# aokomoriuta/ConjugateGradient

Hardware: AMD Instinct MI355X
Metric: CG iterations/sec (7-pt Poisson 512^3); SpMV achieved HBM GB/s in roofline (higher is better)
Workload: dtype f64

## Files before the change

### conjugategradient_amd/csrc/common.hpp

```cpp
#pragma once
#include <hip/hip_runtime.h>
#include <cstddef>
#include <cstdint>
#include <cstdio>
#include <cstdarg>
#include <cstring>
#include <cmath>
#include <atomic>
#include <mutex>
#include <string>
#include <type_traits>
#include <vector>

#pragma GCC visibility push(default)
#include "../../include/MgcgGpu.h"
#pragma GCC visibility pop

namespace mgcg {

constexpr int kWave = 64;
constexpr int kBlock = 256;
constexpr int kNumXcd = 8;
constexpr int kNumCu = 256;
constexpr int kMaxGrid = kNumCu * 8;
// ... 580 lines not shown
void lsqr_enqueue_v(const LsqrRun& R, const FinalizeArgs& f, int k, int nUU);
int lsqr_enqueue_close_residual(const LsqrRun& R);
int lsqr_enqueue_close_normal(const LsqrRun& R);

int launch_cheb_start(hipStream_t s, const double* r, const double* dinv, double* d, double* z, long long n, double it,
                      double* partials, double* partialsZ, bool withRz);
void launch_cheb_init_scalars(hipStream_t s, const double* partials, int n, const double* partialsZ, int nZ, bool reduceFirst, const FinalizeArgs& f);
int launch_cheb_first(hipStream_t s, const FinalizeArgs& f, double* r, const double* Ap, const double* dinv, double* d, double* z, long long n, double it,
                      double* partials, double* partialsZ, bool withRz, const double* pApPartials, int nPAp);
void launch_cheb_finalize(hipStream_t s, const double* partials, int n, const double* partialsZ, int nZ, bool reduceFirst, const FinalizeArgs& f);
void launch_gershgorin(hipStream_t s, const double* elements, const int* rowOffsets, long long nnz, long long n, const double* dinv, double* partials, double* out);

void launch_jacobi_setup(hipStream_t s, const double* elements, const int* rowOffsets, const int* columnIndeces, long long nnz, long long n, long long rowBase,
                         double* dinv, int* bad );

struct FinalizeArgs {
    CgScalars* sc;
    HostMirror* mirror;
    double* trace; int traceCap;
    double tol; int minIt; int maxIt; int rule;
    int preconditioned;
};
struct StopDecision { double res, shown; bool stop; int status; };
__device__ __forceinline__ StopDecision decide_stop(const FinalizeArgs& f, double rrNew, double inf, double rr0, int it)
{
    StopDecision d;
    d.res = sqrt(rrNew);
    if (f.rule == MGCG_RULE_HANDMADECL) d.res = inf;
    d.shown = d.res;
    bool converged;
    switch (f.rule) {
    case MGCG_RULE_NATIVE:   converged = (f.minIt <= it) && (d.res < f.tol); break;
    case MGCG_RULE_SIMPLE:   converged = (f.minIt < it) && (d.res < f.tol); break;
    case MGCG_RULE_VIENNACL: d.shown = sqrt(rrNew / rr0); converged = (f.minIt < it) && (rrNew / rr0 < f.tol * f.tol); break;
    default:                 converged = (it >= f.minIt) && (it <= f.maxIt) && (d.res < f.tol); break;
    }
    d.status = MGCG_OK;
    d.stop = converged;
    if (!d.stop && it >= f.minIt && it > f.maxIt) { d.stop = true; d.status = MGCG_MAXIT_EXCEEDED; }
    if (!d.stop && !(d.res == d.res && fabs(d.res) <= 1.79e308)) { d.stop = true; d.status = MGCG_NONFINITE; }
    return d;
}
void launch_reduce_to(hipStream_t s, const double* partials, int n, double* dst, const int* done);
void launch_reduce2_to(hipStream_t s, const double* pA, int nA, double* dstA, const double* pB, int nB, double* dstB, const int* done);
void launch_finalize(hipStream_t s, const double* partials, const double* partialsInf, int n, bool reduceFirst, const FinalizeArgs& f);
void launch_finalize_precond(hipStream_t s, const double* partials, int n, bool reduceFirst, CgScalars* sc);
void launch_init_scalars(hipStream_t s, const double* partials, const double* partialsZ, int n, bool reduceFirst, CgScalars* sc, HostMirror* mirror);

void launch_jacobi_first(hipStream_t s, long long n, double omega, const double* dinv, int dinvUniform, double dinvScalar, const double* b, double* x, const int* done);
void launch_uniform_check(hipStream_t s, const double* v, long long n, int* flag);
void launch_restrict(hipStream_t s, int nx, int ny, int nz, const double* r, double* bc, const int* done);
void launch_prolong_add(hipStream_t s, int nx, int ny, int nz, double* x, const double* e, const int* done);
void launch_prolong_linear_add(hipStream_t s, int nx, int ny, int nz, int z0, int z1, double* x, const double* eFull, const int* done);
void launch_restrict_linear(hipStream_t s, int nx, int ny, int nz, int z0, int z1, const double* rFull, double* bc, const int* done);
void launch_prolong_scaled(hipStream_t s, int nx, int ny, int nz, double* x, const double* b, double inner, double outer, const double* e, const int* done);
void launch_extract_dinv(hipStream_t s, const double* elements, const int* rowOffsets, const int* columnIndeces,
                         long long n, long long rowBase, double* dinv);
void launch_galerkin(hipStream_t s, int nx, int ny, int nz, int zBegin, int zEnd, const double* elements, const int* rowOffsets, const int* columnIndeces,
                     double sigma, const int* rowOffsetsC, int* countsC, double* elementsC, int* columnIndecesC, int* errFlag);
void launch_poisson(hipStream_t s, int nx, int ny, int nz, int zBegin, int zEnd, double* elements, int* rowOffsets, int* columnIndeces);
void launch_rebase(hipStream_t s, int* rowOffsets, long long n, int base);
long long poisson_nnz_host(int nx, int ny, int nz, int zBegin, int zEnd);
void launch_minmax_int(hipStream_t s, const int* v, long long n, int* out2 );
void launch_halo_rows(hipStream_t s, const int* rowOffsets, const int* columnIndeces, long long n, long long offset, int* out2 );

void launch_amg_restrict(hipStream_t s, long long nc, const int* aggOffsets, const int* members, const double* r, double* bc, const int* done);
void launch_amg_prolong_add(hipStream_t s, long long n, const int* agg, double* x, const double* e, const int* done);
void launch_amg_check_diagonal(hipStream_t s, const double* elements, const int* rowOffsets, const int* columnIndeces, long long n, int* badRow);
void launch_amg_row_max(hipStream_t s, const double* elements, const int* rowOffsets, const int* columnIndeces, long long n, double* rowMax);
void launch_amg_match_round(hipStream_t s, const double* elements, const int* rowOffsets, const int* columnIndeces, long long n, double theta,
                            const double* rowMax, int* match, int* pick, int* flags2);
void launch_amg_galerkin_count(hipStream_t s, long long nc, const int* aggOffsets, const int* members, const int* rowOffsets, const int* columnIndeces,
                               const int* agg, const int* expandOffsets, int* scratch, int* counts);
void launch_amg_galerkin_fill(hipStream_t s, long long nc, const int* aggOffsets, const int* members, const double* elements, const int* rowOffsets,
                              const int* columnIndeces, const int* agg, const int* expandOffsets, const int* scratch, const int* rowOffsetsC, double sigma,
                              double* elementsC, int* columnIndecesC);
void launch_amg_gather_values(hipStream_t s, long long m, const int* source, const double* elements, double* out);

constexpr int kTransposeShortMax = 32;
constexpr int kTransposeLdsMax = 4096;
void launch_transpose_check_offsets(hipStream_t s, const int* rowOffsets, long long rows, int* status3);
void launch_transpose_count(hipStream_t s, const int* rowOffsets, const int* columnIndeces, long long rows, long long columns, long long nnz, int* counts, int* badRow);
bool launch_transpose_claim_and_sort(hipStream_t s, const int* rowOffsets, const int* columnIndeces, long long rows, long long columns, long long nnz,
                                     const int* offsetsT, int* cursor, int* work, unsigned long long* keys);
void launch_transpose_emit(hipStream_t s, long long nnz, const unsigned long long* keys, const double* elements, int* outColumns, int* outSource, double* outElements);
void launch_transpose_merged(hipStream_t s, const int* rowOffsets, const int* columnIndeces, const int* offsetsT, const unsigned long long* keys, long long n, long long nnz,
                             int* mergedOffsets, int* mergedColumns, int* mergedSource);
void preload_kernels_transpose();

void launch_gs_colour_round(hipStream_t s, const int* rowOffsets, const int* columnIndeces, long long n, const int* colourIn, int* colourOut, int* flags, int* badRow);
void launch_gs_check(hipStream_t s, const int* rowOffsets, const int* columnIndeces, long long n, const int* colour, int* badRow);
void launch_gs_zero(hipStream_t s, long long n, double* x, const int* done);
void launch_gs_sweep(hipStream_t s, const int* rows, int count, const double* elements, const int* rowOffsets, const int* columnIndeces,
                     const double* b, const double* dinv, double omega, double* x, double avgRow, const int* done);
void preload_kernels_gs();

void launch_ilu_check_rows(hipStream_t s, const int* rowOffsets, const int* columnIndeces, long long n, int* flags3);
void launch_ilu_lengths(hipStream_t s, const int* rowOffsets, const int* rowOf, long long n, int* lengths);
void launch_ilu_build(hipStream_t s, const double* elements, const int* rowOffsets, const int* columnIndeces, const int* rowOf, const int* newOf, long long n,
                      double shift, const int* offsetsB, double* valuesB, int* columnsB, int* diagPos, int* dupRow, int lanes);
void launch_ilu_factor(hipStream_t s, int row0, int count, const int* offsetsB, const int* columnsB, const int* diagPos, double* valuesB, double* pinv,
                       const int* rowOf, int* badRow, int lanes);
int launch_ilu_pivot_range(hipStream_t s, const double* valuesB, const int* diagPos, long long n, double* partials);
void launch_ilu_pass(hipStream_t s, bool backward, int row0, int count, const double* valuesB, const int* offsetsB, const int* columnsB, const int* diagPos,
                     const double* pinv, const int* rowOf, const double* r, double* y, double* t, double* z, int lanes, const int* done);
void preload_kernels_ilu();
// ... 23 lines not shown
```

### conjugategradient_amd/csrc/kernels_mg.hip

```cpp
#include "common.hpp"

namespace mgcg {

static inline int grid1(long long n)
{
    long long b = (n + kBlock - 1) / kBlock;
    if (b > kMaxGrid) b = kMaxGrid;
    if (b < 1) b = 1;
    return (int)b;
}

typedef double d2mg __attribute__((ext_vector_type(2)));

template <bool UNIFORM>
__global__ __launch_bounds__(kBlock) void jacobi_first_kernel(long long n, double omega, const double* __restrict__ dinv, double dscalar,
                                                              const double* __restrict__ b, double* __restrict__ x, const int* done)
{
    if (done != nullptr && *done != 0) return;
    const bool wide = ((((uintptr_t)b) | ((uintptr_t)x) | ((uintptr_t)dinv)) & 15) == 0;
    if (wide) {
        const long long n2 = n >> 1;
        const long long per = ((n2 + gridDim.x - 1) / gridDim.x + (kBlock - 1)) & ~(long long)(kBlock - 1);
        long long end = per * (blockIdx.x + 1);
        end = end < n2 ? end : n2;
// ... 99 lines not shown
    const long long pairsL = (long long)(nx / 2) * ny * nz;
    if (pairsL <= 0 || pairsL >= 0x7fffffffLL) return false;
    const unsigned half = (unsigned)nx / 2, pairs = (unsigned)pairsL;
    auto lg = [](unsigned v) { int l = 0; while ((1u << l) < v) ++l; return ((1u << l) == v) ? l : -1; };
    const int lgHalf = lg(half), lgNy = lg((unsigned)ny);
    const bool pow2 = lgHalf >= 0 && lgNy >= 0;
    const int cy = ny > 1 ? 2 : 1, cz = nz > 1 ? 2 : 1;
    const unsigned NX = half, NY = (unsigned)(ny / cy);
    const int grid = grid1((long long)pairs);
#define GO(S, P) hipLaunchKernelGGL((prolong_pairs_kernel<S, P>), dim3(grid), dim3(kBlock), 0, s, half, (unsigned)ny, lgHalf, lgNy, cy, cz, NX, NY, pairs, x, b, inner, outer, e, done)
    if (scaled) { if (pow2) GO(true, true); else GO(true, false); }
    else { if (pow2) GO(false, true); else GO(false, false); }
#undef GO
    return true;
}

void launch_prolong_add(hipStream_t s, int nx, int ny, int nz, double* x, const double* e, const int* done)
{
    if (launch_prolong_pairs(s, false, nx, ny, nz, x, x, 0.0, 0.0, e, done)) return;
    hipLaunchKernelGGL(prolong_add_kernel, dim3(grid1((long long)nx * ny * nz)), dim3(kBlock), 0, s, nx, ny, nz, x, e, done);
}

__global__ __launch_bounds__(kBlock) void prolong_scaled_kernel(int nx, int ny, int nz, double* __restrict__ x, const double* __restrict__ b,
                                                                double inner, double outer, const double* __restrict__ e, const int* done)
{
    if (done != nullptr && *done != 0) return;
    const int cx = nx > 1 ? 2 : 1, cy = ny > 1 ? 2 : 1, cz = nz > 1 ? 2 : 1;
    const int NX = nx / cx, NY = ny / cy;
    const long long N = (long long)nx * ny * nz;
    const long long stride = (long long)gridDim.x * kBlock;
    for (long long i = (long long)blockIdx.x * kBlock + threadIdx.x; i < N; i += stride) {
        const int xx = (int)(i % nx), yy = (int)((i / nx) % ny), zz = (int)(i / ((long long)nx * ny));
        const double t = inner * b[i];
        const double x1 = outer * t;
        x[i] = x1 + e[((long long)(zz / cz) * NY + (yy / cy)) * NX + (xx / cx)];
    }
}
void launch_prolong_scaled(hipStream_t s, int nx, int ny, int nz, double* x, const double* b, double inner, double outer, const double* e, const int* done)
{
    if (launch_prolong_pairs(s, true, nx, ny, nz, x, b, inner, outer, e, done)) return;
    hipLaunchKernelGGL(prolong_scaled_kernel, dim3(grid1((long long)nx * ny * nz)), dim3(kBlock), 0, s, nx, ny, nz, x, b, inner, outer, e, done);
}

__device__ __forceinline__ int lin_terms(int i, int n, int idx[2], double w[2])
{
    if (n == 1) { idx[0] = 0; w[0] = 1.0; return 1; }
    const int I = i >> 1, J = (i & 1) ? I + 1 : I - 1;
    idx[0] = I; w[0] = 0.75;
    if (J < 0 || J >= (n >> 1)) return 1;
    idx[1] = J; w[1] = 0.25;
    return 2;
}

__global__ __launch_bounds__(kBlock) void prolong_linear_add_kernel(int nx, int ny, int nz, int z0, int z1, double* __restrict__ x,
                                                                    const double* __restrict__ eFull, const int* done)
{
    if (done != nullptr && *done != 0) return;
    const int NX = nx > 1 ? nx / 2 : 1, NY = ny > 1 ? ny / 2 : 1;
    const long long N = (long long)nx * ny * (z1 - z0);
    const long long stride = (long long)gridDim.x * kBlock;
    for (long long i = (long long)blockIdx.x * kBlock + threadIdx.x; i < N; i += stride) {
        const int xx = (int)(i % nx), yy = (int)((i / nx) % ny), zz = z0 + (int)(i / ((long long)nx * ny));
        int iz[2], iy[2], ix[2]; double wz[2], wy[2], wx[2];
        const int kz = lin_terms(zz, nz, iz, wz), ky = lin_terms(yy, ny, iy, wy), kx = lin_terms(xx, nx, ix, wx);
        double sum = 0.0;
        for (int a = 0; a < kz; ++a)
            for (int b = 0; b < ky; ++b) {
                const double wzy = wz[a] * wy[b];
                const long long base = ((long long)iz[a] * NY + iy[b]) * NX;
                for (int c = 0; c < kx; ++c) { const double w = wzy * wx[c]; const double t = w * eFull[base + ix[c]]; sum += t; }
            }
        x[i] = x[i] + sum;
    }
}
__global__ __launch_bounds__(kBlock) void prolong_linear_add_rows_kernel(int nx, int ny, int nz, int z0, int z1, int tx, double* __restrict__ x,
                                                                         const double* __restrict__ eFull, const int* done)
{
    if (done != nullptr && *done != 0) return;
    const int NX = nx >> 1, NY = ny > 1 ? ny / 2 : 1;
    const int ty = kBlock / tx;
    const int lx = threadIdx.x % tx, ly = threadIdx.x / tx;
    const long long rows = (long long)ny * (z1 - z0);
    const long long band = (rows + 7) / 8;
    const long long bandBegin = (blockIdx.x & 7) * band, bandEnd = bandBegin + band < rows ? bandBegin + band : rows;
    for (long long row = bandBegin + (long long)(blockIdx.x >> 3) * ty + ly; row < bandEnd; row += (long long)(gridDim.x >> 3) * ty) {
        const unsigned r32 = (unsigned)row;
        const int yy = (int)(r32 % (unsigned)ny), zz = z0 + (int)(r32 / (unsigned)ny);
        int iz[2], iy[2]; double wz[2], wy[2];
        const int kz = lin_terms(zz, nz, iz, wz), ky = lin_terms(yy, ny, iy, wy);
        d2mg* xr = (d2mg*)(x + row * nx);
        if (kz == 1) { iz[1] = iz[0]; wz[1] = 0.0; }
        if (ky == 1) { iy[1] = iy[0]; wy[1] = 0.0; }
        for (int X = lx; X < NX; X += tx) {
            const bool hasL = X > 0, hasR = X + 1 < NX;
            const int XL = hasL ? X - 1 : X, XR = hasR ? X + 1 : X;
            double eC[4], eL[4], eR[4];
#pragma unroll
            for (int t = 0; t < 4; ++t) {
                const double* er = eFull + ((long long)iz[t >> 1] * NY + iy[t & 1]) * NX;
                eC[t] = er[X]; eL[t] = er[XL]; eR[t] = er[XR];
            }
            double sumL = 0.0, sumR = 0.0;
#pragma unroll
            for (int t = 0; t < 4; ++t) {
                const bool term = (t >> 1) < kz && (t & 1) < ky;
                const double wzy = wz[t >> 1] * wy[t & 1];
                const double w3 = wzy * 0.75, w1 = wzy * 0.25;
                const double pC = w3 * eC[t], pL = w1 * eL[t], pR = w1 * eR[t];
                const double tC = term ? pC : 0.0;
                sumL += tC; sumR += tC;
                sumL += (term && hasL) ? pL : 0.0;
                sumR += (term && hasR) ? pR : 0.0;
            }
            d2mg v = xr[X];
            v.x = v.x + sumL; v.y = v.y + sumR;
            xr[X] = v;
        }
    }
}
static int rows_tx(int pairs) { int t = 1; while (t < pairs && t < kBlock) t <<= 1; return t; }
void launch_prolong_linear_add(hipStream_t s, int nx, int ny, int nz, int z0, int z1, double* x, const double* eFull, const int* done)
{
    if (nx >= 2 && (nx & 1) == 0 && (((uintptr_t)x) & 15) == 0) {
        const int tx = rows_tx(nx / 2), ty = kBlock / tx;
        const long long rows = (long long)ny * (z1 - z0);
        long long g = ((rows + 7) / 8 + ty - 1) / ty * 8; if (g > kMaxGrid) g = kMaxGrid; if (g < 8) g = 8;
        hipLaunchKernelGGL(prolong_linear_add_rows_kernel, dim3((int)g), dim3(kBlock), 0, s, nx, ny, nz, z0, z1, tx, x, eFull, done);
        return;
    }
    hipLaunchKernelGGL(prolong_linear_add_kernel, dim3(grid1((long long)nx * ny * (z1 - z0))), dim3(kBlock), 0, s, nx, ny, nz, z0, z1, x, eFull, done);
}

__global__ __launch_bounds__(kBlock) void restrict_linear_kernel(int nx, int ny, int nz, int z0, int z1, const double* __restrict__ rFull,
                                                                 double* __restrict__ bc, const int* done)
{
    if (done != nullptr && *done != 0) return;
    const int cz = nz > 1 ? 2 : 1;
    const int NX = nx > 1 ? nx / 2 : 1, NY = ny > 1 ? ny / 2 : 1;
    const int Z0 = z0 / cz, ZL = (z1 - z0) / cz;
    const long long NC = (long long)NX * NY * ZL;
    const long long stride = (long long)gridDim.x * kBlock;
    for (long long I = (long long)blockIdx.x * kBlock + threadIdx.x; I < NC; I += stride) {
        const int X = (int)(I % NX), Y = (int)((I / NX) % NY), Z = Z0 + (int)(I / ((long long)NX * NY));
        auto span = [](int C, int n, int& first, int& count, int& quarterFirst) {
            if (n == 1) { first = 0; count = 1; quarterFirst = -1; return; }
            const int lo = 2 * C - 1, hi = 2 * C + 2;
            first = lo < 0 ? 0 : lo; count = (hi >= n ? n - 1 : hi) - first + 1; quarterFirst = lo < 0 ? 0 : 1;
        };
        int fz, nzT, qz, fy, nyT, qy, fx, nxT, qx;
        span(Z, nz, fz, nzT, qz); span(Y, ny, fy, nyT, qy); span(X, nx, fx, nxT, qx);
        auto weight = [](int k, int q) { if (q < 0) return 1.0; const int rel = k + (1 - q); return (rel == 0 || rel == 3) ? 0.25 : 0.75; };
        double sum = 0.0;
        for (int a = 0; a < nzT; ++a) {
            const double wza = weight(a, qz);
            for (int b = 0; b < nyT; ++b) {
                const double wzy = wza * weight(b, qy);
                const long long base = ((long long)(fz + a) * ny + (fy + b)) * nx + fx;
                for (int c = 0; c < nxT; ++c) { const double w = wzy * weight(c, qx); const double t = w * rFull[base + c]; sum += t; }
            }
        }
        bc[I] = sum;
    }
}
__global__ __launch_bounds__(kBlock) void restrict_linear_rows_kernel(int nx, int ny, int nz, int z0, int z1, int tx, const double* __restrict__ rFull,
                                                                      double* __restrict__ bc, const int* done)
{
    if (done != nullptr && *done != 0) return;
    const int cz = nz > 1 ? 2 : 1;
    const int NX = nx >> 1, NY = ny > 1 ? ny / 2 : 1;
    const int Z0 = z0 / cz, ZL = (z1 - z0) / cz;
    const int ty = kBlock / tx;
    const int lx = threadIdx.x % tx, ly = threadIdx.x / tx;
    const long long rows = (long long)NY * ZL;
    auto span = [](int C, int n, int& first, int& count, int& quarterFirst) {
        if (n == 1) { first = 0; count = 1; quarterFirst = -1; return; }
        const int lo = 2 * C - 1, hi = 2 * C + 2;
        first = lo < 0 ? 0 : lo; count = (hi >= n ? n - 1 : hi) - first + 1; quarterFirst = lo < 0 ? 0 : 1;
    };
    auto weight = [](int k, int q) { if (q < 0) return 1.0; const int rel = k + (1 - q); return (rel == 0 || rel == 3) ? 0.25 : 0.75; };
    const long long band = (rows + 7) / 8;
    const long long bandBegin = (blockIdx.x & 7) * band, bandEnd = bandBegin + band < rows ? bandBegin + band : rows;
    for (long long row = bandBegin + (long long)(blockIdx.x >> 3) * ty + ly; row < bandEnd; row += (long long)(gridDim.x >> 3) * ty) {
        const unsigned r32 = (unsigned)row;
        const int Y = (int)(r32 % (unsigned)NY), Z = Z0 + (int)(r32 / (unsigned)NY);
        int fz, nzT, qz, fy, nyT, qy;
        span(Z, nz, fz, nzT, qz); span(Y, ny, fy, nyT, qy);
        for (int X = lx; X < NX; X += tx) {
            const bool hasL = X > 0, hasR = 2 * X + 2 < nx;
            const int oL = hasL ? -1 : 0, oR = hasR ? 2 : 0;
            double sum = 0.0;
#pragma unroll
            for (int a0 = 0; a0 < 4; a0 += 2) {
                d2mg mid[8]; double left[8], right[8];
#pragma unroll
                for (int t = 0; t < 8; ++t) {
                    const int a = a0 + (t >> 2), b = t & 3;
                    const int za = a < nzT ? a : 0, yb = b < nyT ? b : 0;
                    const double* rr = rFull + ((long long)(fz + za) * ny + (fy + yb)) * nx + 2 * X;
                    mid[t] = *(const d2mg*)rr; left[t] = rr[oL]; right[t] = rr[oR];
                }
#pragma unroll
                for (int t = 0; t < 8; ++t) {
                    const int a = a0 + (t >> 2), b = t & 3;
                    const bool term = a < nzT && b < nyT;
                    const double wzy = weight(a, qz) * weight(b, qy);
                    const double w3 = wzy * 0.75, w1 = wzy * 0.25;
                    const double pl = w1 * left[t], p0 = w3 * mid[t].x, p1 = w3 * mid[t].y, pr = w1 * right[t];
                    sum += (term && hasL) ? pl : 0.0;
                    sum += term ? p0 : 0.0;
                    sum += term ? p1 : 0.0;
                    sum += (term && hasR) ? pr : 0.0;
                }
            }
            bc[row * NX + X] = sum;
        }
    }
}
void launch_restrict_linear(hipStream_t s, int nx, int ny, int nz, int z0, int z1, const double* rFull, double* bc, const int* done)
{
    if (nx >= 2 && (nx & 1) == 0 && (((uintptr_t)rFull) & 15) == 0) {
        const int tx = rows_tx(nx / 2), ty = kBlock / tx;
        const long long rows = (long long)(ny > 1 ? ny / 2 : 1) * ((z1 - z0) / (nz > 1 ? 2 : 1));
        long long g = ((rows + 7) / 8 + ty - 1) / ty * 8; if (g > kMaxGrid) g = kMaxGrid; if (g < 8) g = 8;
        hipLaunchKernelGGL(restrict_linear_rows_kernel, dim3((int)g), dim3(kBlock), 0, s, nx, ny, nz, z0, z1, tx, rFull, bc, done);
        return;
    }
    const long long NC = (long long)(nx > 1 ? nx / 2 : 1) * (ny > 1 ? ny / 2 : 1) * ((z1 - z0) / (nz > 1 ? 2 : 1));
    hipLaunchKernelGGL(restrict_linear_kernel, dim3(grid1(NC)), dim3(kBlock), 0, s, nx, ny, nz, z0, z1, rFull, bc, done);
}

__global__ __launch_bounds__(kBlock) void extract_dinv_kernel(const double* __restrict__ elements, const int* __restrict__ rowOffsets,
                                                              const int* __restrict__ columnIndeces, long long n, long long rowBase, double* __restrict__ dinv)
{
    const long long stride = (long long)gridDim.x * kBlock;
    for (long long i = (long long)blockIdx.x * kBlock + threadIdx.x; i < n; i += stride) {
        double d = 0.0;
        for (int k = rowOffsets[i]; k < rowOffsets[i + 1]; ++k)
            if (columnIndeces[k] == rowBase + i) { d = elements[k]; break; }
        dinv[i] = 1.0 / d;
    }
}
void launch_extract_dinv(hipStream_t s, const double* elements, const int* rowOffsets, const int* columnIndeces,
                         long long n, long long rowBase, double* dinv)
{
    hipLaunchKernelGGL(extract_dinv_kernel, dim3(grid1(n)), dim3(kBlock), 0, s, elements, rowOffsets, columnIndeces, n, rowBase, dinv);
}

__global__ __launch_bounds__(kBlock) void galerkin_kernel(int nx, int ny, int nz, int zBegin, int zEnd,
                                                          const double* __restrict__ elements, const int* __restrict__ rowOffsets,
                                                          const int* __restrict__ columnIndeces, double sigma, const int* __restrict__ rowOffsetsC,
                                                          int* __restrict__ countsC, double* __restrict__ elementsC, int* __restrict__ columnIndecesC, int* errFlag)
{
    const int cx = nx > 1 ? 2 : 1, cy = ny > 1 ? 2 : 1, cz = nz > 1 ? 2 : 1;
    const int NX = nx / cx, NY = ny / cy;
    const int ZL = (zEnd - zBegin) / cz;
    const int Z0 = zBegin / cz;
    const long long NC = (long long)NX * NY * ZL;
    const long long sxy = (long long)nx * ny;
    const long long stride = (long long)gridDim.x * kBlock;
    for (long long I = (long long)blockIdx.x * kBlock + threadIdx.x; I < NC; I += stride) {
        const int X = (int)(I % NX), Y = (int)((I / NX) % NY), Zl = (int)(I / ((long long)NX * NY));
        const int Z = Z0 + Zl;
        double acc[27];
        unsigned touched = 0u;
#pragma unroll
        for (int q = 0; q < 27; ++q) acc[q] = 0.0;
        for (int dz = 0; dz < cz; ++dz)
            for (int dy = 0; dy < cy; ++dy)
                for (int dx = 0; dx < cx; ++dx) {
                    const long long i = ((long long)(Zl * cz + dz) * ny + (Y * cy + dy)) * nx + (X * cx + dx);
                    for (int k = rowOffsets[i]; k < rowOffsets[i + 1]; ++k) {
                        const long long j = columnIndeces[k];
                        const int jx = (int)(j % nx), jy = (int)((j / nx) % ny), jz = (int)(j / sxy);
                        const int ox = jx / cx - X, oy = jy / cy - Y, oz = jz / cz - Z;
                        if (ox < -1 || ox > 1 || oy < -1 || oy > 1 || oz < -1 || oz > 1) { *errFlag = 1; continue; }
                        const int q = (oz + 1) * 9 + (oy + 1) * 3 + (ox + 1);
                        const double v = elements[k];
// ... 149 lines not shown
```

### conjugategradient_amd/csrc/solver.hip

```cpp
#include "common.hpp"
#include <algorithm>
#include <chrono>
#include <functional>

namespace mgcg {

struct MgLevel {
    int nx = 0, ny = 0, nz = 0;
    int z0 = 0, z1 = 0;
    long long n = 0, nnz = 0;
    long long nGlobal = 0, offset = 0;
    double* elements = nullptr; int* rowOffsets = nullptr; int* columnIndeces = nullptr;
    bool ownsMatrix = false;
    double* dinv = nullptr;
    bool dinvUniform = false; double dinvScalar = 0.0;
    double *xa = nullptr, *xb = nullptr;
    double *b = nullptr, *r = nullptr;
    SpmvConfig cfg;
    const DcsrMatrix* dcsr = nullptr;
    HaloPlan* halo = nullptr;
    HaloPlan* transferHalo = nullptr;
    int minJ = 0, maxJ = -1;
    bool overlap = false;
    long long interior0 = 0, interior1 = 0;
// ... 252 lines not shown
        SpmvArgs f{};
        f.elements = L.extElements; f.rowOffsets = L.extRowOffsets; f.columnIndeces = L.extColumnIndeces; f.x = L.bFull; f.y = L.xb + L.extBase;
        f.elementsCount = (int)L.extNnz; f.rowCount = (int)L.extRows; f.columnCount = (int)L.nGlobal;
        f.w = nullptr; f.b = L.bFull + L.extBase; f.dinv = L.extDinv; f.dinvUniform = 1; f.dinvScalar = L.dinvScalar; f.omega = mg->omega; f.doneFlag = done;
        f.xScaled = 2; f.xInner = L.dinvScalar; f.xOuter = mg->omega; f.xCoarse = e;
        const int lx = log2_exact(L.nx), ly = log2_exact(L.ny), sy = L.ny > 1 ? 1 : 0, sz = L.nz > 1 ? 1 : 0;
        f.cM0 = L.nx / 2 - 1; f.cS1 = 1 + sy; f.cM1 = ((L.ny >> sy) - 1) << (lx - 1);
        f.cS2 = 1 + sy + sz; f.cM2 = (int)(~0u << (lx - 1 + ly - sy));
        f.cRowBase = (int)L.extBase;
        (void)launch_spmv_range(s, EPI_JACOBI, f, L.cfg, nullptr, r0, r1, nullptr, 0);
        *result = L.xb;
        return true;
    }
    const int za = zlo(2), zb = zhi(2);
    launch_prolong_add(s, L.nx, L.ny, zb - za, L.xa + (long long)za * plane, e + (long long)(za / 2) * C.nx * C.ny, done);
    sweep(1, L.xa, L.xb);
    *result = L.xb;
    return true;
}

static void mg_deep_prolong_halo(MgcgMg* mg, MgLevel& L, MgLevel& C, double* cur, const double* e, const int* done)
{
    const long long plane = (long long)L.nx * L.ny, cplane = (long long)C.nx * C.ny;
    if (L.z0 > 0) launch_prolong_add(mg->stream, L.nx, L.ny, 1, cur + (long long)(L.z0 - 1) * plane, e + (long long)((L.z0 - 1) / 2) * cplane, done);
    if (L.z1 < L.nz) launch_prolong_add(mg->stream, L.nx, L.ny, 1, cur + (long long)L.z1 * plane, e + (long long)(L.z1 / 2) * cplane, done);
}

static bool mg_vcycle(MgcgMg* mg, int l, const double* b, double* x0, double* x1, const int* done, double** result)
{
    MgLevel& L = mg->lv[l];
    if (l == mg->levels - 1) return mg_smooth(mg, L, b, x0, x1, mg->nuCoarse, true, done, result, l == 0);
    MgLevel& C = mg->lv[l + 1];
    double* cur = nullptr;
    if (L.agg != nullptr) {
        if (!mg_smooth(mg, L, b, x0, x1, mg->nu, true, done, &cur)) return false;
        double* spare = (cur == x0) ? x1 : x0;
        SpmvArgs ar{};
        ar.elements = L.elements; ar.rowOffsets = L.rowOffsets; ar.columnIndeces = L.columnIndeces; ar.x = cur; ar.y = L.r;
        ar.elementsCount = (int)L.nnz; ar.rowCount = (int)L.n; ar.columnCount = (int)L.nGlobal; ar.b = b; ar.doneFlag = done;
        if (!mg_spmv(mg, L, EPI_RESIDUAL, ar, cur)) return false;
        launch_amg_restrict(mg->stream, C.n, L.aggOffsets, L.aggMembers, L.r, C.b, done);
        double* ec = nullptr;
        if (!mg_vcycle(mg, l + 1, C.b, C.xa, C.xb, done, &ec)) return false;
        launch_amg_prolong_add(mg->stream, L.n, L.agg, cur, ec, done);
        return mg_smooth(mg, L, b, cur, spare, mg->nu, false, done, result, l == 0);
    }
    const bool linear = mg->interp == 1;
    bool canScale = false;
    if (L.dcsr != nullptr && L.dcsr->usable) canScale = L.dcsr->patternId != nullptr;
    else {
        SpmvArgs probe{}; probe.elements = L.elements; probe.columnIndeces = L.columnIndeces; probe.elementsCount = (int)L.nnz; probe.rowCount = (int)L.n;
        canScale = spmv_takes_rowtile(probe, L.cfg);
    }
    const bool mayFold = mg->nu == 1 && !linear && L.dinvUniform && canScale && tuning().noFold.load(std::memory_order_relaxed) == 0;
    const bool fold = mayFold && !mg->multi;
    if (l == 0 && mg->deep && mg->deep0 && mg->rExt != nullptr && b == mg->rExt + (long long)L.nx * L.ny && mayFold && (L.dcsr == nullptr || !L.dcsr->usable) &&
        L.nx >= 2 && log2_exact(L.nx) >= 1 && log2_exact(L.ny) >= 0 && L.nGlobal < 0x7fffffffLL && tuning().foldUp.load(std::memory_order_relaxed) != 0) {
        SpmvArgs a{};
        a.elements = L.elements; a.rowOffsets = L.rowOffsets; a.columnIndeces = L.columnIndeces; a.x = b - L.offset; a.y = L.r;
        a.elementsCount = (int)L.nnz; a.rowCount = (int)L.n; a.columnCount = (int)L.nGlobal; a.b = b; a.doneFlag = done;
        a.xScaled = 1; a.xInner = L.dinvScalar; a.xOuter = mg->omega;
        if (!mg_spmv(mg, L, EPI_RESIDUAL, a, const_cast<double*>(b) - L.offset)) return false;
        launch_restrict(mg->stream, L.nx, L.ny, L.z1 - L.z0, L.r, C.b, done);
        double* e = nullptr;
        if (!mg_deep_level(mg, 1, done, &e)) return false;
        t_lastFolds |= 1 | 2 | 4 | 8;
        struct SkipHalo { MgcgMg* m; ~SkipHalo() { m->skipHalo = false; } } skip{ mg };
        mg->skipHalo = true;
        if (!mg_jacobi(mg, L, b, x0, x1, done, true, e, false, true)) return false;
        *result = x1;
        return true;
    }
    const long long plane = (long long)L.nx * L.ny;
    const long long zoneLo = L.interior0 > 0 ? L.interior0 + 2 * plane : 0;
    const long long zoneHi = L.interior1 < L.n ? L.interior1 - 2 * plane : L.n;
    const bool foldInterior = mayFold && mg->multi && (L.dcsr == nullptr || !L.dcsr->usable) && zoneLo <= zoneHi && 2 * (L.interior1 - L.interior0) >= L.n &&
                              (L.n >= 3000000 || tuning().overlap.load(std::memory_order_relaxed) == 2);
    if (fold || foldInterior) t_lastFolds |= 1;
    if (fold) cur = x0;
    else if (foldInterior) {
        cur = x0;
        if (zoneLo > 0) launch_jacobi_first(mg->stream, zoneLo, mg->omega, L.dinv, 1, L.dinvScalar, b, cur + L.offset, done);
        if (zoneHi < L.n) launch_jacobi_first(mg->stream, L.n - zoneHi, mg->omega, L.dinv, 1, L.dinvScalar, b + zoneHi, cur + L.offset + zoneHi, done);
    }
    else if (!mg_smooth(mg, L, b, x0, x1, mg->nu, true, done, &cur)) return false;
    double* other = (cur == x0) ? x1 : x0;
    SpmvArgs a{};
    const bool rFullLength = linear && mg->multi;
    a.elements = L.elements; a.rowOffsets = L.rowOffsets; a.columnIndeces = L.columnIndeces; a.x = fold ? b : cur; a.y = rFullLength ? other + L.offset : L.r;
    a.elementsCount = (int)L.nnz; a.rowCount = (int)L.n; a.columnCount = (int)L.nGlobal; a.b = b; a.doneFlag = done;
    if (fold) { a.xScaled = 1; a.xInner = L.dinvScalar; a.xOuter = mg->omega; }
    if (foldInterior) {
        SpmvArgs ai = a;
        ai.x = b - L.offset;
        ai.xScaled = 1; ai.xInner = L.dinvScalar; ai.xOuter = mg->omega;
        if (!mg_spmv2(mg, L, EPI_RESIDUAL, ai, a, cur, nullptr, nullptr, true)) return false;
    }
    else if (!mg_spmv(mg, L, EPI_RESIDUAL, a, cur)) return false;
    if (linear) {
        if (rFullLength && !halo_exchange(mg->comm, L.transferHalo, other, mg->stream)) return false;
        launch_restrict_linear(mg->stream, L.nx, L.ny, L.nz, L.z0, L.z1, rFullLength ? other : L.r, C.b, done);
    } else {
        launch_restrict(mg->stream, L.nx, L.ny, L.z1 - L.z0, L.r, C.b, done);
    }
    double* e = nullptr;
    const bool deep = mg->deep && !linear && l == 0;
    if (deep) { if (!mg_deep_level(mg, 1, done, &e)) return false; t_lastFolds |= 4; }
    else if (!mg_vcycle(mg, l + 1, C.b, C.xa, C.xb, done, &e)) return false;
    struct SkipHalo { MgcgMg* m; bool on; ~SkipHalo() { if (on) m->skipHalo = false; } } skip{ mg, deep };
    if (linear) {
        if (mg->multi && !halo_exchange(mg->comm, C.transferHalo, e, mg->stream)) return false;
        launch_prolong_linear_add(mg->stream, L.nx, L.ny, L.nz, L.z0, L.z1, cur + L.offset, e, done);
    }
    else if (fold && (L.dcsr == nullptr || !L.dcsr->usable) && L.nx >= 2 && log2_exact(L.nx) >= 1 && log2_exact(L.ny) >= 0 && L.nGlobal < 0x7fffffffLL &&
             (tuning().foldUp.load(std::memory_order_relaxed) < 0 ? L.n <= kFoldUpMaxRows : tuning().foldUp.load(std::memory_order_relaxed) != 0)) {
        if (!mg_jacobi(mg, L, b, cur, other, done, l == 0, e + C.offset)) return false;
        t_lastFolds |= 2;
        *result = other;
        return true;
    }
    else if (foldInterior && L.nx >= 2 && log2_exact(L.nx) >= 1 && log2_exact(L.ny) >= 0 && L.nGlobal < 0x7fffffffLL && L.nz > 1 && (L.z0 & 1) == 0 && ((L.z1 - L.z0) & 1) == 0 &&
             (tuning().foldUp.load(std::memory_order_relaxed) < 0 ? L.n <= kFoldUpMaxRows : tuning().foldUp.load(std::memory_order_relaxed) != 0)) {
        const long long planes = L.z1 - L.z0, coarsePlane = (long long)C.nx * C.ny;
        const long long loPlanes = zoneLo / plane;
        long long hiStart = zoneHi / plane;
        if (hiStart & 1) --hiStart;
        if (hiStart < loPlanes) {
            launch_prolong_scaled(mg->stream, L.nx, L.ny, (int)planes, cur + L.offset, b, L.dinvScalar, mg->omega, e + C.offset, done);
        } else {
            if (loPlanes > 0) launch_prolong_scaled(mg->stream, L.nx, L.ny, (int)loPlanes, cur + L.offset, b, L.dinvScalar, mg->omega, e + C.offset, done);
            if (zoneHi < L.n) {
                const long long r0 = hiStart * plane;
                launch_prolong_scaled(mg->stream, L.nx, L.ny, (int)(planes - hiStart), cur + L.offset + r0, b + r0, L.dinvScalar, mg->omega,
                                      e + C.offset + (hiStart / 2) * coarsePlane, done);
            }
        }
        if (deep) { mg_deep_prolong_halo(mg, L, C, cur, e, done); mg->skipHalo = true; }
        if (!mg_jacobi(mg, L, b, cur, other, done, l == 0, e, true)) return false;
        t_lastFolds |= 2;
        *result = other;
        return true;
    }
    else if (fold || foldInterior) launch_prolong_scaled(mg->stream, L.nx, L.ny, L.z1 - L.z0, cur + L.offset, b, L.dinvScalar, mg->omega, e + C.offset, done);
    else launch_prolong_add(mg->stream, L.nx, L.ny, L.z1 - L.z0, cur + L.offset, e + C.offset, done);
    if (deep) { mg_deep_prolong_halo(mg, L, C, cur, e, done); mg->skipHalo = true; }
    return mg_smooth(mg, L, b, cur, other, mg->nu, false, done, result, l == 0);
}

static bool mg_apply(MgcgMg* mg, const double* r, double* z, const int* done, double* dotPartials = nullptr, int* nDot = nullptr)
{
    mg->fuseDotPartials = dotPartials; mg->fusedDotCount = 0;
    t_lastFolds = 0;
    struct Reset { MgcgMg* m; int* n; ~Reset() { if (n) *n = m->fusedDotCount; m->fuseDotPartials = nullptr; } } reset{ mg, nDot };
    MgLevel& L0 = mg->lv[0];
    if (mg->ilu != nullptr) {
        const MgIlu& F = *mg->ilu;
        const int colours = (int)F.colourOffsets.size() - 1;
        for (int pass = 0; pass < 2; ++pass)
            for (int q = 0; q < colours; ++q) {
                const int c = pass == 0 ? q : colours - 1 - q;
                launch_ilu_pass(mg->stream, pass == 1, F.colourOffsets[(size_t)c], F.colourOffsets[(size_t)c + 1] - F.colourOffsets[(size_t)c], F.values, F.offsets,
                                F.columns, F.diag, F.pinv, F.rowOf, r, L0.xa, L0.xb, z, F.lanes, done);
            }
        return MGCG_HIP(hipGetLastError());
    }
// ... 3169 lines not shown
```

Measured before the change: 269.2.

## Tile linear prolong/restrict with LDS ring buffers and fold Jacobi scaling into prolong

Replaces the row-based linear prolongation and restriction kernels with 3D-tiled kernels. Each block streams z-planes of the coarse or fine grid through a shared-memory ring, so neighbouring values are reused from LDS instead of being re-read from global memory. It also adds a scaled prolongation variant that, when folding is allowed, computes x = omega*dinv*b + P e directly. This skips reading the old x on linear-interpolation levels. The cost is extra synchronisation, LDS pressure and a more complex tile-to-block mapping.

```diff
diff --git a/conjugategradient_amd/csrc/common.hpp b/conjugategradient_amd/csrc/common.hpp
--- a/conjugategradient_amd/csrc/common.hpp
+++ b/conjugategradient_amd/csrc/common.hpp
@@ -656,6 +656,8 @@
 void launch_restrict(hipStream_t s, int nx, int ny, int nz, const double* r, double* bc, const int* done);
 void launch_prolong_add(hipStream_t s, int nx, int ny, int nz, double* x, const double* e, const int* done);
 void launch_prolong_linear_add(hipStream_t s, int nx, int ny, int nz, int z0, int z1, double* x, const double* eFull, const int* done);
+void launch_prolong_linear_scaled(hipStream_t s, int nx, int ny, int nz, int z0, int z1, double* x, const double* b, double inner, double outer,
+                                  const double* eFull, const int* done);
 void launch_restrict_linear(hipStream_t s, int nx, int ny, int nz, int z0, int z1, const double* rFull, double* bc, const int* done);
 void launch_prolong_scaled(hipStream_t s, int nx, int ny, int nz, double* x, const double* b, double inner, double outer, const double* e, const int* done);
 void launch_extract_dinv(hipStream_t s, const double* elements, const int* rowOffsets, const int* columnIndeces,
diff --git a/conjugategradient_amd/csrc/kernels_mg.hip b/conjugategradient_amd/csrc/kernels_mg.hip
--- a/conjugategradient_amd/csrc/kernels_mg.hip
+++ b/conjugategradient_amd/csrc/kernels_mg.hip
@@ -175,7 +175,9 @@
     return 2;
 }
 
+template <bool SCALED>
 __global__ __launch_bounds__(kBlock) void prolong_linear_add_kernel(int nx, int ny, int nz, int z0, int z1, double* __restrict__ x,
+                                                                    const double* __restrict__ b, double inner, double outer,
                                                                     const double* __restrict__ eFull, const int* done)
 {
     if (done != nullptr && *done != 0) return;
@@ -188,70 +190,123 @@
         const int kz = lin_terms(zz, nz, iz, wz), ky = lin_terms(yy, ny, iy, wy), kx = lin_terms(xx, nx, ix, wx);
         double sum = 0.0;
         for (int a = 0; a < kz; ++a)
-            for (int b = 0; b < ky; ++b) {
-                const double wzy = wz[a] * wy[b];
-                const long long base = ((long long)iz[a] * NY + iy[b]) * NX;
-                for (int c = 0; c < kx; ++c) { const double w = wzy * wx[c]; const double t = w * eFull[base + ix[c]]; sum += t; }
+            for (int c = 0; c < ky; ++c) {
+                const double wzy = wz[a] * wy[c];
+                const long long base = ((long long)iz[a] * NY + iy[c]) * NX;
+                for (int d = 0; d < kx; ++d) { const double w = wzy * wx[d]; const double t = w * eFull[base + ix[d]]; sum += t; }
             }
-        x[i] = x[i] + sum;
-    }
-}
-__global__ __launch_bounds__(kBlock) void prolong_linear_add_rows_kernel(int nx, int ny, int nz, int z0, int z1, int tx, double* __restrict__ x,
-                                                                         const double* __restrict__ eFull, const int* done)
-{
-    if (done != nullptr && *done != 0) return;
-    const int NX = nx >> 1, NY = ny > 1 ? ny / 2 : 1;
-    const int ty = kBlock / tx;
-    const int lx = threadIdx.x % tx, ly = threadIdx.x / tx;
-    const long long rows = (long long)ny * (z1 - z0);
-    const long long band = (rows + 7) / 8;
-    const long long bandBegin = (blockIdx.x & 7) * band, bandEnd = bandBegin + band < rows ? bandBegin + band : rows;
-    for (long long row = bandBegin + (long long)(blockIdx.x >> 3) * ty + ly; row < bandEnd; row += (long long)(gridDim.x >> 3) * ty) {
-        const unsigned r32 = (unsigned)row;
-        const int yy = (int)(r32 % (unsigned)ny), zz = z0 + (int)(r32 / (unsigned)ny);
-        int iz[2], iy[2]; double wz[2], wy[2];
-        const int kz = lin_terms(zz, nz, iz, wz), ky = lin_terms(yy, ny, iy, wy);
-        d2mg* xr = (d2mg*)(x + row * nx);
-        if (kz == 1) { iz[1] = iz[0]; wz[1] = 0.0; }
-        if (ky == 1) { iy[1] = iy[0]; wy[1] = 0.0; }
-        for (int X = lx; X < NX; X += tx) {
-            const bool hasL = X > 0, hasR = X + 1 < NX;
-            const int XL = hasL ? X - 1 : X, XR = hasR ? X + 1 : X;
-            double eC[4], eL[4], eR[4];
+        double x1;
+        if (SCALED) { const double t = inner * b[i]; x1 = outer * t; } else x1 = x[i];
+        x[i] = x1 + sum;
+    }
+}
+
+constexpr int kTileX = 64, kTileY = 4, kTileZ = 32;
+static_assert(kTileX * kTileY == kBlock, "one lane per coarse cell of a tile");
+struct TileGrid { int tilesX, tilesY, chunks, zc, per; };
+static bool tile_grid(int nx, int ny, int nz, int z0, int z1, TileGrid* g)
+{
+    const int cz = nz > 1 ? 2 : 1, NX = nx / 2, NY = ny > 1 ? ny / 2 : 1, ZL = (z1 - z0) / cz;
+    if (ZL < 1 || z0 % cz != 0 || (z1 - z0) % cz != 0) return false;
+    g->tilesX = (NX + kTileX - 1) / kTileX; g->tilesY = (NY + kTileY - 1) / kTileY;
+    g->zc = kTileZ;
+    while (g->zc > 1 && (long long)g->tilesX * g->tilesY * ((ZL + g->zc - 1) / g->zc) < 4 * kNumCu) g->zc >>= 1;
+    g->chunks = (ZL + g->zc - 1) / g->zc;
+    const long long total = (long long)g->tilesX * g->tilesY * g->chunks;
+    if (total > 0x3fffffffLL) return false;
+    g->per = (int)((total + 7) / 8);
+    return true;
+}
+__device__ __forceinline__ bool tile_of_block(const TileGrid& g, int* tX, int* tY, int* chunk)
+{
+    const long long t = (long long)(blockIdx.x & 7) * g.per + (blockIdx.x >> 3);
+    if (t >= (long long)g.tilesX * g.tilesY * g.chunks) return false;
+    *tX = (int)(t % g.tilesX); *tY = (int)((t / g.tilesX) % g.tilesY); *chunk = (int)(t / ((long long)g.tilesX * g.tilesY));
+    return true;
+}
+
+template <bool SCALED>
+__global__ __launch_bounds__(kBlock) void prolong_linear_tiles_kernel(int nx, int ny, int nz, int z0, int z1, TileGrid g, double* __restrict__ x,
+                                                                      const double* __restrict__ b, double inner, double outer,
+                                                                      const double* __restrict__ eFull, const int* done)
+{
+    if (done != nullptr && *done != 0) return;
+    __shared__ double ring[4][kTileY + 2][kTileX + 2];
+    int tX, tY, chunk;
+    if (!tile_of_block(g, &tX, &tY, &chunk)) return;
+    const int cy = ny > 1 ? 2 : 1, cz = nz > 1 ? 2 : 1;
+    const int NX = nx >> 1, NY = ny / cy, NZ = nz / cz;
+    const int X0 = tX * kTileX, Y0 = tY * kTileY;
+    const int Zb = z0 / cz + chunk * g.zc, ZeAll = z0 / cz + (z1 - z0) / cz, Ze = Zb + g.zc < ZeAll ? Zb + g.zc : ZeAll;
+    const int lx = threadIdx.x & (kTileX - 1), lr = threadIdx.x / kTileX;
+    const int X = X0 + lx;
+    const bool hasL = X > 0, hasR = X + 1 < NX;
+    const int rowsShift = cy == 2 ? 3 : 2;
+    static_assert(kTileY == 4, "rowsShift");
+    int loaded = 0;
+    for (int Z = Zb; Z < Ze; ++Z) {
+        const int needLo = Z - (cz - 1) < 0 ? 0 : Z - (cz - 1), needHi = Z + (cz - 1) > NZ - 1 ? NZ - 1 : Z + (cz - 1);
+        for (int P = (Z == Zb ? needLo : loaded); P <= needHi; ++P)
+            for (int q = threadIdx.x; q < (kTileY + 2) * (kTileX + 2); q += kBlock) {
+                const int j = q / (kTileX + 2), i = q - j * (kTileX + 2);
+                const int Yc = Y0 - 1 + j, Xc = X0 - 1 + i;
+                const bool in = Yc >= 0 && Yc < NY && Xc >= 0 && Xc < NX;
+                ring[P & 3][j][i] = in ? eFull[((long long)P * NY + Yc) * NX + Xc] : 0.0;
+            }
+        loaded = needHi + 1;
+        __syncthreads();
+        if (X >= NX) continue;
+        for (int u = lr; u < cz * cy * kTileY; u += kBlock / kTileX) {
+            const int zz = cz * Z + (u >> rowsShift), yy = cy * Y0 + (u & ((1 << rowsShift) - 1));
+            if (yy >= ny) continue;
+            int iz[2], iy[2]; double wz[2], wy[2];
+            const int kz = lin_terms(zz, nz, iz, wz), ky = lin_terms(yy, ny, iy, wy);
+            if (kz == 1) { iz[1] = iz[0]; wz[1] = 0.0; }
+            if (ky == 1) { iy[1] = iy[0]; wy[1] = 0.0; }
+            double sumL = 0.0, sumR = 0.0;
 #pragma unroll
             for (int t = 0; t < 4; ++t) {
-                const double* er = eFull + ((long long)iz[t >> 1] * NY + iy[t & 1]) * NX;
-                eC[t] = er[X]; eL[t] = er[XL]; eR[t] = er[XR];
-            }
-            double sumL = 0.0, sumR = 0.0;
-#pragma unroll
-            for (int t = 0; t < 4; ++t) {
+                const double* er = &ring[iz[t >> 1] & 3][iy[t & 1] - (Y0 - 1)][lx];
+                const double eL = er[0], eC = er[1], eR = er[2];
                 const bool term = (t >> 1) < kz && (t & 1) < ky;
                 const double wzy = wz[t >> 1] * wy[t & 1];
                 const double w3 = wzy * 0.75, w1 = wzy * 0.25;
-                const double pC = w3 * eC[t], pL = w1 * eL[t], pR = w1 * eR[t];
+                const double pC = w3 * eC, pL = w1 * eL, pR = w1 * eR;
                 const double tC = term ? pC : 0.0;
                 sumL += tC; sumR += tC;
                 sumL += (term && hasL) ? pL : 0.0;
                 sumR += (term && hasR) ? pR : 0.0;
             }
-            d2mg v = xr[X];
+            const long long row = (long long)(zz - z0) * ny + yy;
+            d2mg* xr = (d2mg*)(x + row * nx);
+            d2mg v = SCALED ? ((const d2mg*)(b + row * nx))[X] : xr[X];
+            if (SCALED) { const double t0 = inner * v.x, t1 = inner * v.y; v.x = outer * t0; v.y = outer * t1; }
             v.x = v.x + sumL; v.y = v.y + sumR;
             xr[X] = v;
         }
     }
 }
-static int rows_tx(int pairs) { int t = 1; while (t < pairs && t < kBlock) t <<= 1; return t; }
+static void launch_prolong_linear(hipStream_t s, bool scaled, int nx, int ny, int nz, int z0, int z1, double* x, const double* b, double inner, double outer,
+                                  const double* eFull, const int* done)
+{
+    TileGrid tg;
+    if (nx >= 2 && (nx & 1) == 0 && ((((uintptr_t)x) | ((uintptr_t)b)) & 15) == 0 && tile_grid(nx, ny, nz, z0, z1, &tg)) {
+        if (scaled) hipLaunchKernelGGL(prolong_linear_tiles_kernel<true>, dim3(8 * tg.per), dim3(kBlock), 0, s, nx, ny, nz, z0, z1, tg, x, b, inner, outer, eFull, done);
+        else hipLaunchKernelGGL(prolong_linear_tiles_kernel<false>, dim3(8 * tg.per), dim3(kBlock), 0, s, nx, ny, nz, z0, z1, tg, x, b, inner, outer, eFull, done);
+        return;
+    }
+    const int grid = grid1((long long)nx * ny * (z1 - z0));
+    if (scaled) hipLaunchKernelGGL(prolong_linear_add_kernel<true>, dim3(grid), dim3(kBlock), 0, s, nx, ny, nz, z0, z1, x, b, inner, outer, eFull, done);
+    else hipLaunchKernelGGL(prolong_linear_add_kernel<false>, dim3(grid), dim3(kBlock), 0, s, nx, ny, nz, z0, z1, x, b, inner, outer, eFull, done);
+}
 void launch_prolong_linear_add(hipStream_t s, int nx, int ny, int nz, int z0, int z1, double* x, const double* eFull, const int* done)
 {
-    if (nx >= 2 && (nx & 1) == 0 && (((uintptr_t)x) & 15) == 0) {
-        const int tx = rows_tx(nx / 2), ty = kBlock / tx;
-        const long long rows = (long long)ny * (z1 - z0);
-        long long g = ((rows + 7) / 8 + ty - 1) / ty * 8; if (g > kMaxGrid) g = kMaxGrid; if (g < 8) g = 8;
-        hipLaunchKernelGGL(prolong_linear_add_rows_kernel, dim3((int)g), dim3(kBlock), 0, s, nx, ny, nz, z0, z1, tx, x, eFull, done);
-        return;
-    }
-    hipLaunchKernelGGL(prolong_linear_add_kernel, dim3(grid1((long long)nx * ny * (z1 - z0))), dim3(kBlock), 0, s, nx, ny, nz, z0, z1, x, eFull, done);
+    launch_prolong_linear(s, false, nx, ny, nz, z0, z1, x, x, 0.0, 0.0, eFull, done);
+}
+void launch_prolong_linear_scaled(hipStream_t s, int nx, int ny, int nz, int z0, int z1, double* x, const double* b, double inner, double outer,
+                                  const double* eFull, const int* done)
+{
+    launch_prolong_linear(s, true, nx, ny, nz, z0, z1, x, b, inner, outer, eFull, done);
 }
 
 __global__ __launch_bounds__(kBlock) void restrict_linear_kernel(int nx, int ny, int nz, int z0, int z1, const double* __restrict__ rFull,
@@ -285,67 +340,105 @@
         bc[I] = sum;
     }
 }
-__global__ __launch_bounds__(kBlock) void restrict_linear_rows_kernel(int nx, int ny, int nz, int z0, int z1, int tx, const double* __restrict__ rFull,
-                                                                      double* __restrict__ bc, const int* done)
-{
-    if (done != nullptr && *done != 0) return;
-    const int cz = nz > 1 ? 2 : 1;
-    const int NX = nx >> 1, NY = ny > 1 ? ny / 2 : 1;
-    const int Z0 = z0 / cz, ZL = (z1 - z0) / cz;
-    const int ty = kBlock / tx;
-    const int lx = threadIdx.x % tx, ly = threadIdx.x / tx;
-    const long long rows = (long long)NY * ZL;
+constexpr int kFineRows = 2 * kTileY + 2, kFinePitch = 2 * kTileX + 4;
+constexpr int kFetchPairs = 2 * kFineRows * kTileX / kBlock;
+static_assert(2 * kFineRows * kTileX % kBlock == 0 && 2 * kFineRows * 2 <= kBlock, "fetch: whole rounds of pairs, one round of edge cells");
+__global__ __launch_bounds__(kBlock) void restrict_linear_tiles_kernel(int nx, int ny, int nz, int z0, int z1, TileGrid g, const double* __restrict__ rFull,
+                                                                       double* __restrict__ bc, const int* done)
+{
+    if (done != nullptr && *done != 0) return;
+    __shared__ __attribute__((aligned(16))) double ring[4][kFineRows][kFinePitch];
+    int tX, tY, chunk;
+    if (!tile_of_block(g, &tX, &tY, &chunk)) return;
+    const int cy = ny > 1 ? 2 : 1, cz = nz > 1 ? 2 : 1;
+    const int NX = nx >> 1, NY = ny / cy;
+    const int X0 = tX * kTileX, Y0 = tY * kTileY;
+    const int Z0 = z0 / cz, Zb = Z0 + chunk * g.zc, ZeAll = Z0 + (z1 - z0) / cz, Ze = Zb + g.zc < ZeAll ? Zb + g.zc : ZeAll;
+    const int lx = threadIdx.x & (kTileX - 1), ly = threadIdx.x / kTileX;
+    const int X = X0 + lx, Y = Y0 + ly;
+    const int rowLo = cy * Y0 - 1;
+    d2mg fp[kFetchPairs]; double fe = 0.0;
+    auto fetch = [&](int pA) {
+#pragma unroll
+        for (int k = 0; k < kFetchPairs; ++k) {
+            const int q = threadIdx.x + k * kBlock;
+            const int p = pA + q / (kFineRows * kTileX), j = (q / kTileX) % kFineRows, i = q % kTileX;
+            const int yr = rowLo + j, col = 2 * (X0 + i);
+            const bool in = p >= 0 && p < nz && yr >= 0 && yr < ny && col < nx;
+            d2mg v; v.x = 0.0; v.y = 0.0;
+            if (in) v = *(const d2mg*)(rFull + ((long long)p * ny + yr) * nx + col);
+            fp[k] = v;
+        }
+        fe = 0.0;
+        if (threadIdx.x < 2 * kFineRows * 2) {
+            const int p = pA + threadIdx.x / (kFineRows * 2), j = (threadIdx.x >> 1) % kFineRows, right = threadIdx.x & 1;
+            const int yr = rowLo + j, col = right ? 2 * (X0 + kTileX) : 2 * X0 - 1;
+            if (p >= 0 && p < nz && yr >= 0 && yr < ny && col >= 0 && col < nx) fe = rFull[((long long)p * ny + yr) * nx + col];
+        }
+    };
+    auto stash = [&](int pA) {
+#pragma unroll
+        for (int k = 0; k < kFetchPairs; ++k) {
+            const int q = threadIdx.x + k * kBlock;
+            const int p = pA + q / (kFineRows * kTileX), j = (q / kTileX) % kFineRows, i = q % kTileX;
+            *(d2mg*)&ring[p & 3][j][2 + 2 * i] = fp[k];
+        }
+        if (threadIdx.x < 2 * kFineRows * 2) {
+            const int p = pA + threadIdx.x / (kFineRows * 2), j = (threadIdx.x >> 1) % kFineRows, right = threadIdx.x & 1;
+            ring[p & 3][j][right ? 2 + 2 * kTileX : 1] = fe;
+        }
+    };
     auto span = [](int C, int n, int& first, int& count, int& quarterFirst) {
         if (n == 1) { first = 0; count = 1; quarterFirst = -1; return; }
         const int lo = 2 * C - 1, hi = 2 * C + 2;
         first = lo < 0 ? 0 : lo; count = (hi >= n ? n - 1 : hi) - first + 1; quarterFirst = lo < 0 ? 0 : 1;
     };
     auto weight = [](int k, int q) { if (q < 0) return 1.0; const int rel = k + (1 - q); return (rel == 0 || rel == 3) ? 0.25 : 0.75; };
-    const long long band = (rows + 7) / 8;
-    const long long bandBegin = (blockIdx.x & 7) * band, bandEnd = bandBegin + band < rows ? bandBegin + band : rows;
-    for (long long row = bandBegin + (long long)(blockIdx.x >> 3) * ty + ly; row < bandEnd; row += (long long)(gridDim.x >> 3) * ty) {
-        const unsigned r32 = (unsigned)row;
-        const int Y = (int)(r32 % (unsigned)NY), Z = Z0 + (int)(r32 / (unsigned)NY);
-        int fz, nzT, qz, fy, nyT, qy;
-        span(Z, nz, fz, nzT, qz); span(Y, ny, fy, nyT, qy);
-        for (int X = lx; X < NX; X += tx) {
-            const bool hasL = X > 0, hasR = 2 * X + 2 < nx;
-            const int oL = hasL ? -1 : 0, oR = hasR ? 2 : 0;
+    const int pFirst = cz == 2 ? 2 * Zb - 1 : -1;
+    fetch(pFirst); stash(pFirst);
+    fetch(pFirst + 2); stash(pFirst + 2);
+    __syncthreads();
+    const bool hasL = X > 0, hasR = 2 * X + 2 < nx;
+    for (int Z = Zb; Z < Ze; ++Z) {
+        const bool more = Z + 1 < Ze;
+        if (more) fetch(2 * Z + 3);
+        if (X < NX && Y < NY) {
+            int fz, nzT, qz, fy, nyT, qy;
+            span(Z, nz, fz, nzT, qz); span(Y, ny, fy, nyT, qy);
             double sum = 0.0;
 #pragma unroll
-            for (int a0 = 0; a0 < 4; a0 += 2) {
-                d2mg mid[8]; double left[8], right[8];
-#pragma unroll
-                for (int t = 0; t < 8; ++t) {
-                    const int a = a0 + (t >> 2), b = t & 3;
-                    const int za = a < nzT ? a : 0, yb = b < nyT ? b : 0;
-                    const double* rr = rFull + ((long long)(fz + za) * ny + (fy + yb)) * nx + 2 * X;
-                    mid[t] = *(const d2mg*)rr; left[t] = rr[oL]; right[t] = rr[oR];
-                }
-#pragma unroll
-                for (int t = 0; t < 8; ++t) {
-                    const int a = a0 + (t >> 2), b = t & 3;
-                    const bool term = a < nzT && b < nyT;
-                    const double wzy = weight(a, qz) * weight(b, qy);
+            for (int a = 0; a < 4; ++a) {
+                const int za = a < nzT ? a : 0;
+#pragma unroll
+                for (int c = 0; c < 4; ++c) {
+                    const int yc = c < nyT ? c : 0;
+                    const double* rr = &ring[(fz + za) & 3][fy + yc - rowLo][2 + 2 * lx];
+                    const d2mg mid = *(const d2mg*)rr;
+                    const double left = rr[-1], right = rr[2];
+                    const bool term = a < nzT && c < nyT;
+                    const double wzy = weight(a, qz) * weight(c, qy);
                     const double w3 = wzy * 0.75, w1 = wzy * 0.25;
-                    const double pl = w1 * left[t], p0 = w3 * mid[t].x, p1 = w3 * mid[t].y, pr = w1 * right[t];
+                    const double pl = w1 * left, p0 = w3 * mid.x, p1 = w3 * mid.y, pr = w1 * right;
                     sum += (term && hasL) ? pl : 0.0;
                     sum += term ? p0 : 0.0;
                     sum += term ? p1 : 0.0;
                     sum += (term && hasR) ? pr : 0.0;
                 }
             }
-            bc[row * NX + X] = sum;
+            bc[((long long)(Z - Z0) * NY + Y) * NX + X] = sum;
+        }
+        if (more) {
+            __syncthreads();
+            stash(2 * Z + 3);
+            __syncthreads();
         }
     }
 }
 void launch_restrict_linear(hipStream_t s, int nx, int ny, int nz, int z0, int z1, const double* rFull, double* bc, const int* done)
 {
-    if (nx >= 2 && (nx & 1) == 0 && (((uintptr_t)rFull) & 15) == 0) {
-        const int tx = rows_tx(nx / 2), ty = kBlock / tx;
-        const long long rows = (long long)(ny > 1 ? ny / 2 : 1) * ((z1 - z0) / (nz > 1 ? 2 : 1));
-        long long g = ((rows + 7) / 8 + ty - 1) / ty * 8; if (g > kMaxGrid) g = kMaxGrid; if (g < 8) g = 8;
-        hipLaunchKernelGGL(restrict_linear_rows_kernel, dim3((int)g), dim3(kBlock), 0, s, nx, ny, nz, z0, z1, tx, rFull, bc, done);
+    TileGrid tg;
+    if (nx >= 2 && (nx & 1) == 0 && (((uintptr_t)rFull) & 15) == 0 && tile_grid(nx, ny, nz, z0, z1, &tg)) {
+        hipLaunchKernelGGL(restrict_linear_tiles_kernel, dim3(8 * tg.per), dim3(kBlock), 0, s, nx, ny, nz, z0, z1, tg, rFull, bc, done);
         return;
     }
     const long long NC = (long long)(nx > 1 ? nx / 2 : 1) * (ny > 1 ? ny / 2 : 1) * ((z1 - z0) / (nz > 1 ? 2 : 1));
diff --git a/conjugategradient_amd/csrc/solver.hip b/conjugategradient_amd/csrc/solver.hip
--- a/conjugategradient_amd/csrc/solver.hip
+++ b/conjugategradient_amd/csrc/solver.hip
@@ -328,8 +328,9 @@
         SpmvArgs probe{}; probe.elements = L.elements; probe.columnIndeces = L.columnIndeces; probe.elementsCount = (int)L.nnz; probe.rowCount = (int)L.n;
         canScale = spmv_takes_rowtile(probe, L.cfg);
     }
-    const bool mayFold = mg->nu == 1 && !linear && L.dinvUniform && canScale && tuning().noFold.load(std::memory_order_relaxed) == 0;
-    const bool fold = mayFold && !mg->multi;
+    const bool foldable = mg->nu == 1 && L.dinvUniform && canScale && tuning().noFold.load(std::memory_order_relaxed) == 0;
+    const bool mayFold = foldable && !linear;
+    const bool fold = foldable && !mg->multi;
     if (l == 0 && mg->deep && mg->deep0 && mg->rExt != nullptr && b == mg->rExt + (long long)L.nx * L.ny && mayFold && (L.dcsr == nullptr || !L.dcsr->usable) &&
         L.nx >= 2 && log2_exact(L.nx) >= 1 && log2_exact(L.ny) >= 0 && L.nGlobal < 0x7fffffffLL && tuning().foldUp.load(std::memory_order_relaxed) != 0) {
         SpmvArgs a{};
@@ -386,7 +387,8 @@
     struct SkipHalo { MgcgMg* m; bool on; ~SkipHalo() { if (on) m->skipHalo = false; } } skip{ mg, deep };
     if (linear) {
         if (mg->multi && !halo_exchange(mg->comm, C.transferHalo, e, mg->stream)) return false;
-        launch_prolong_linear_add(mg->stream, L.nx, L.ny, L.nz, L.z0, L.z1, cur + L.offset, e, done);
+        if (fold) launch_prolong_linear_scaled(mg->stream, L.nx, L.ny, L.nz, L.z0, L.z1, cur + L.offset, b, L.dinvScalar, mg->omega, e, done);
+        else launch_prolong_linear_add(mg->stream, L.nx, L.ny, L.nz, L.z0, L.z1, cur + L.offset, e, done);
     }
     else if (fold && (L.dcsr == nullptr || !L.dcsr->usable) && L.nx >= 2 && log2_exact(L.nx) >= 1 && log2_exact(L.ny) >= 0 && L.nGlobal < 0x7fffffffLL &&
              (tuning().foldUp.load(std::memory_order_relaxed) < 0 ? L.n <= kFoldUpMaxRows : tuning().foldUp.load(std::memory_order_relaxed) != 0)) {
```

Measured after the change: 263.1. -2.3%, worse.
